# Yelp/nrtsearch

Hardware: AMD Instinct MI355X
Metric: queries/sec, 10M-doc 5-term BM25 top-1000 (higher is better)
Workload: dtype f32

## Files before the change

nrtsearch_amd/csrc/kernels.hip:

```cpp
#include <hip/hip_runtime.h>
#include <stdint.h>

#include "bm25_common.hiph"

namespace nrtgpu {

struct ScanSmem {
  uint64_t acc[kScanWaves][kTileDocs];
  uint64_t cand[kCandCap];
  uint32_t tab[kTabTerms][kTabEntries];
  float    cache[kLdsCaches][256];
  alignas(16) uint32_t w_incl[kScanWaves][kMaxTerms];
  alignas(16) uint32_t w_rec[kScanWaves][kMaxTerms][4];
  uint32_t w_before[kScanWaves][kMaxTerms];
  TopkScratch sc;
  uint64_t theta;
  uint64_t thr;
  uint32_t cnt;
  uint32_t tile_cand;
  uint32_t slot_hits[kSliceSlots];
  uint32_t slot_slice[kSliceSlots];
  uint32_t rz_flag;
  uint32_t cnt_valid;
  uint32_t next_tile;
// ... 714 lines not shown
      hits += h;
      if (h != 0u && q.gte_floor != 0xFFFFFFFFu) atomicAdd(&slice_sum[q.slice_base + s.slot_slice[i]], h);
    }
    item_hits[blockIdx.x] = hits;
    if (ABL == 7 && item_prof) {
      s.prof[4] += __builtin_readcyclecounter() - t_epi;
      for (int i = 0; i < 16; ++i) item_prof[(size_t)blockIdx.x * 16 + i] = s.prof[i];
    }
  }
}

struct MergeSmem {
  uint64_t cand[kMergeCap];
  TopkScratch sc;
  uint64_t theta;
  unsigned long long hits;
  uint32_t cnt;
  uint32_t pad;
  uint32_t lrec[kScanThreads];
  uint32_t loff[kScanThreads + 1];
  uint32_t wtot[kScanThreads / 64];
};

__device__ __noinline__ void merge_compact(MergeSmem& s, uint32_t n, uint32_t k) {
  uint64_t thr = 0;
  const uint32_t m = topk_compact<kScanThreads, kMergeCap>(s.cand, n, k, &s.sc, &thr);
  if (n > k && threadIdx.x == 0) {
    s.cnt = m;
    if (thr > s.theta) s.theta = thr;
  }
  __syncthreads();
}

__global__ __launch_bounds__(kScanThreads)
void merge_topk_kernel(const uint64_t* __restrict__ in_keys, const uint32_t* __restrict__ in_counts,
                       const uint64_t* __restrict__ in_hits, const uint32_t* __restrict__ list_idx,
                       const uint32_t* __restrict__ q_base, const uint32_t* __restrict__ q_nlists, uint32_t k_stride_in,
                       const uint32_t* __restrict__ q_k, uint64_t* __restrict__ out_keys,
                       uint32_t* __restrict__ out_counts, uint64_t* __restrict__ out_hits,
                       uint32_t k_stride_out, const uint32_t* __restrict__ help_query, uint32_t n_help,
                       uint32_t help_slot_base, const unsigned long long* __restrict__ spec_g) {
  __shared__ MergeSmem s;
  const uint32_t tid = threadIdx.x;
  const uint32_t q = blockIdx.x;
  const uint32_t k = q_k[q];
  const uint32_t nl = q_nlists[q];
  const uint32_t base = q_base[q];
  if (tid == 0) {
    s.theta = 0;
    s.hits = 0;
    s.cnt = 0;
  }
  __syncthreads();
  const uint32_t n_lists = nl + (help_query ? n_help : 0u);
  for (uint32_t l0 = 0; l0 < n_lists; l0 += kScanThreads) {
    const uint32_t l = l0 + tid;
    uint32_t rec = 0xFFFFFFFFu, c = 0;
    if (l < nl) {
      rec = list_idx[base + l];
    } else if (l < n_lists && help_query[l - nl] == q + 1u) {
      rec = help_slot_base + (l - nl);
    }
    if (rec != 0xFFFFFFFFu) {
      c = min(in_counts[rec], k_stride_in);
      const unsigned long long h = in_hits[rec];
      if (h) atomicAdd(&s.hits, h);
    }
    const uint32_t incl = scan64_dpp(c);
    const uint32_t lane = tid & 63u, wave = tid >> 6;
    if (lane == 63u) s.wtot[wave] = incl;
    __syncthreads();
    uint32_t before = 0, total = 0;
    for (uint32_t w = 0; w < (uint32_t)(kScanThreads / 64); ++w) {
      const uint32_t t = s.wtot[w];
      before += w < wave ? t : 0u;
      total += t;
    }
    s.lrec[tid] = rec;
    s.loff[tid] = before + incl - c;
    if (tid == 0) s.loff[kScanThreads] = total;
    __syncthreads();
    for (uint32_t i0 = 0; i0 < total; i0 += kScanThreads) {
      const uint32_t i = i0 + tid;
      uint64_t key = 0;
      bool want = false;
      if (i < total) {
        uint32_t lo = 0, hi = kScanThreads;
        while (hi - lo > 1u) {
          const uint32_t mid = (lo + hi) >> 1;
          if (s.loff[mid] <= i) lo = mid; else hi = mid;
        }
        key = in_keys[(size_t)s.lrec[lo] * k_stride_in + (i - s.loff[lo])];
        want = key > s.theta;
      }
      topk_append(s.cand, &s.cnt, want, key);
      __syncthreads();
      const uint32_t cn = s.cnt;
      __syncthreads();
      if (cn > (uint32_t)(kMergeCap - kScanThreads)) merge_compact(s, cn, k);
    }
    __syncthreads();
  }
  __syncthreads();
  {
    const uint32_t c = s.cnt;
    __syncthreads();
    if (c > k) merge_compact(s, c, k);
// ... 175 lines not shown
void launch_pack_write(hipStream_t stream, const uint32_t* docids, const uint32_t* fnorm, uint64_t n, uint32_t n_blocks,
                       const uint32_t* dir, uint32_t* exceptions, uint32_t* packed) {
  if (n_blocks == 0) return;
  hipLaunchKernelGGL(pack_write_kernel, dim3(n_blocks), dim3(256), 0, stream, docids, fnorm, n, dir, exceptions, packed);
}
void launch_apply_live(hipStream_t stream, const uint32_t* docids, uint32_t* fnorm, uint64_t n, const uint64_t* live) {
  if (n == 0) return;
  const uint64_t blocks = (n + 1023) / 1024;
  hipLaunchKernelGGL(apply_live_kernel, dim3((uint32_t)(blocks < 8192 ? blocks : 8192)), dim3(256), 0, stream, docids, fnorm, n, live);
}
void launch_bm25_scan(hipStream_t stream, bool fixed_point, bool pipelined, bool packed, int ablation, uint32_t n_items, const DItem* items,
                      const DPart* parts, const DTerm* terms, const DQuery* queries, const float* caches, unsigned long long* theta_g,
                      unsigned long long* quant_g, const DExchange* xch, uint32_t* slice_sum, uint64_t* item_keys, uint32_t* item_counts,
                      uint64_t* item_hits, uint32_t k_stride, uint64_t* item_prof) {
  if (n_items == 0) return;
#define NRT_LAUNCH_K(F, P, A, K)                                                                                  \
  hipLaunchKernelGGL((bm25_scan_kernel<F, P, A, K>), dim3(n_items), dim3(kScanThreads), 0, stream, items, parts, terms, queries, \
                     caches, theta_g, quant_g, xch, slice_sum, item_keys, item_counts, item_hits, k_stride, item_prof)
#define NRT_LAUNCH(F, P, A)                 \
  do {                                      \
    if (packed) NRT_LAUNCH_K(F, P, A, true);  \
    else NRT_LAUNCH_K(F, P, A, false);      \
  } while (0)
#define NRT_LAUNCH_FX(P, A)            \
  do {                                 \
    if (fixed_point) NRT_LAUNCH(true, P, A); \
    else NRT_LAUNCH(false, P, A);      \
  } while (0)
  if (ablation == 8) { NRT_LAUNCH(true, true, 8); return; }
  if (ablation == 9) { NRT_LAUNCH_FX(true, 9); return; }
  if (!pipelined) { NRT_LAUNCH_FX(false, 0); return; }
  switch (ablation) {
#ifdef NRTGPU_DEV
    case 1: NRT_LAUNCH_K(false, true, 1, false); break;
    case 2: NRT_LAUNCH_K(false, true, 2, false); break;
    case 3: NRT_LAUNCH_K(false, true, 3, false); break;
    case 4: NRT_LAUNCH_K(false, true, 4, false); break;
    case 6: NRT_LAUNCH_K(false, true, 6, false); break;
    case 7: NRT_LAUNCH_FX(true, 7); break;
#endif
    default: NRT_LAUNCH_FX(true, 0); break;
  }
#undef NRT_LAUNCH_FX
#undef NRT_LAUNCH
#undef NRT_LAUNCH_K
}

void launch_merge_topk(hipStream_t stream, uint32_t n_queries, const uint64_t* in_keys, const uint32_t* in_counts,
                       const uint64_t* in_hits, const uint32_t* list_idx, const uint32_t* q_base,
                       const uint32_t* q_nlists, uint32_t k_stride_in, const uint32_t* q_k, uint64_t* out_keys,
                       uint32_t* out_counts, uint64_t* out_hits, uint32_t k_stride_out, const uint32_t* help_query,
                       uint32_t n_help, uint32_t help_slot_base, const unsigned long long* spec_g) {
  if (n_queries == 0) return;
  hipLaunchKernelGGL(merge_topk_kernel, dim3(n_queries), dim3(kScanThreads), 0, stream, in_keys, in_counts, in_hits,
                     list_idx, q_base, q_nlists, k_stride_in, q_k, out_keys, out_counts, out_hits, k_stride_out, help_query, n_help,
                     help_slot_base, spec_g);
}

void launch_fold_norms(hipStream_t stream, const uint32_t* docids, const uint32_t* freqs, const uint8_t* norms,
                       uint32_t* fnorm, uint64_t n, uint32_t* overflow) {
  if (n == 0) return;
  const uint64_t blocks = (n + 255) / 256;
  hipLaunchKernelGGL(fold_norms_kernel, dim3((uint32_t)(blocks < 4096 ? blocks : 4096)), dim3(256), 0, stream, docids,
                     freqs, norms, fnorm, n, overflow);
}

}
```

nrtsearch_amd/csrc/maxscore.hip:

```cpp
#include <hip/hip_runtime.h>
#include <stdint.h>

#include "bm25_common.hiph"

namespace nrtgpu {

constexpr int kMsWinWords = kMsWinDocs / 32;
constexpr int kSl = kMsSlots;
typedef uint32_t u32x2 __attribute__((ext_vector_type(2)));
typedef const NRT_GLOBAL u32x2* gvec2_ptr;

struct alignas(16) WClause {
  uint64_t docids, fnorm;
  uint64_t begin;
  uint32_t count, pad0;
  float    weight;
  int32_t  fx_scale;
  uint32_t flags;
  uint32_t pad;
  uint64_t u_after;
  uint64_t look;
  uint64_t cells, start;
};
static_assert(sizeof(WClause) == 80, "WClause layout");

struct MsSmem {
  uint64_t cand[kMsCandCap];
  uint32_t tab[kTabTerms][kTabEntries];
  float    cache[kLdsCaches][256];
  uint32_t seen[kMsWaves][kMsWinWords];
  WClause  wc[kMsWaves][kMsMaxTerms];
  TopkScratch sc;
  uint64_t theta;
  uint64_t thr;
  uint32_t cnt;
  uint32_t cnt_valid;
  uint32_t rz_flag;
  uint32_t wins_started;
  uint32_t spec_at;
  uint32_t q_wins;
  uint32_t spec_z16;
  uint32_t spec_grow16;
  unsigned long long* spec_slot;
  uint64_t pick;
  uint32_t role[4];
  uint32_t prune_on;
  uint32_t slot_hits[kSliceSlots];
  uint32_t slot_slice[kSliceSlots];
  uint64_t prof[16];
};
static_assert(sizeof(MsSmem) <= 160 * 1024, "the MaxScore workgroup owns one CU's 160 KiB LDS");

__device__ __forceinline__ uint64_t uniform_u64(uint64_t v) {
  const uint32_t lo = (uint32_t)__builtin_amdgcn_readfirstlane((int)(uint32_t)v);
  const uint32_t hi = (uint32_t)__builtin_amdgcn_readfirstlane((int)(uint32_t)(v >> 32));
  return ((uint64_t)hi << 32) | (uint64_t)lo;
}
__device__ __forceinline__ uint64_t readlane_u64(uint64_t v, uint32_t l) {
  const uint32_t lo = (uint32_t)__builtin_amdgcn_readlane((int)(uint32_t)v, (int)l);
  const uint32_t hi = (uint32_t)__builtin_amdgcn_readlane((int)(uint32_t)(v >> 32), (int)l);
  return ((uint64_t)hi << 32) | (uint64_t)lo;
}

template <bool PACKED, int NS>
__device__ __forceinline__ void values_of_codes(const MsSmem& s, const uint32_t (&c)[NS], uint32_t need, uint32_t tab_slot,
                                                float w, int fx_scale, uint32_t cache_slot, uint64_t esc_list,
                                                const uint32_t (&pidx)[NS], uint32_t (&val)[NS]) {
  const uint32_t tab = tab_slot < (uint32_t)kTabTerms ? tab_slot : 7u;
  const char* tb = (const char*)&s.tab[tab == 7u ? 0u : tab][0];
  uint32_t cor = 0;
#pragma unroll
  for (int j = 0; j < NS; ++j) {
    val[j] = *(const uint32_t*)(tb + (c[j] & 0x1FFCu));
    const uint32_t cn = ((need >> j) & 1u) ? c[j] : 0u;
    cor = PACKED ? max(cor, cn) : (cor | cn);
  }
  const bool special = need != 0u && ((PACKED ? cor >= (kPackEscBase << 2) : (cor >> 31) != 0u) || tab == 7u);
  if (__any(special)) {
    const float* cache = &s.cache[cache_slot][0];
#pragma unroll
    for (int j = 0; j < NS; ++j) {
      uint32_t cj = c[j];
      if (PACKED && cj >= (kPackEscBase << 2)) cj = ((need >> j) & 1u) ? packed_escape_word((gu32_ptr)esc_list, pidx[j], cj >> 2) : 0x80000100u;
      const bool esc = (cj >> 31) != 0u;
      const uint32_t f = esc ? ((cj >> 8) & 0x3FFFFFu) : ((cj >> 9) & 15u);
      const bool dead = esc ? ((cj >> 30) & 1u) != 0u : (cj >> 20) != 0u;
      const uint32_t nb = esc ? (cj & 255u) : ((cj >> 2) & 127u);
      if (((need >> j) & 1u) && (esc || tab == 7u))
        val[j] = dead ? 0u : score_value<true>(bm25_score(w, (float)(int32_t)f, cache[nb]), fx_scale);
    }
  }
}

#ifdef NRT_MS_PHASE_CLOCKS
#define NRT_PH_MARK(i)                                                          \
  do {                                                                          \
    if (PROF) {                                                                 \
      asm volatile("s_waitcnt vmcnt(0) lgkmcnt(0)" ::: "memory");               \
      const uint64_t t_ph_ = __builtin_readcyclecounter();                      \
      ph[i] += t_ph_ - ph_t;                                                    \
      ph_t = t_ph_;                                                             \
    }                                                                           \
  } while (0)
#else
// ... 356 lines not shown
        if (lane < n_terms) my_ub = (uint64_t)ub_raw << mt.fx_shift;
      }
      uint64_t my_after = 0;
      {
        uint64_t run = 0;
        for (int m = (int)n_terms - 1; m >= 0; --m) {
          const uint64_t ub = readlane_u64(my_ub, (uint32_t)m);
          if (lane == (uint32_t)m) my_after = run;
          run = use_max ? max(run, ub) : run + ub;
          if (lane == (uint32_t)m) my_suf = run;
        }
      }
      const gu32_ptr my_cells = (gu32_ptr)mt.cell_off;
      const uint32_t my_shift = mt.shift;
      if (lane < n_terms) {
        WClause w;
        w.docids = (uint64_t)mt.docids;
        w.fnorm = (uint64_t)mt.fnorm;
        w.begin = 0;
        w.count = w.pad0 = 0;
        w.weight = mt.weight;
        w.fx_scale = mt.fx_scale;
        const DTermAux* const ax = mt.aux;
        const uint32_t look_kind = ax->look_kind;
        w.flags = ((mt.tab_slot & 0xFFFFu) < (uint32_t)kTabTerms ? (mt.tab_slot & 0xFFFFu) : 7u) | (TWO && (mt.tab_slot & kTabSlotRequired) ? 8u : 0u) |
                  (mt.fx_shift << 4) | (mt.cache_slot << 8) | ((mt.shift & 31u) << 16) | ((look_kind & 7u) << 24) | (((uint32_t)ax->look_shift & 31u) << 27);
        w.pad = 0;
        w.u_after = my_after;
        w.look = look_kind != kLookNone ? (uint64_t)ax->look : 0ull;
        w.cells = (uint64_t)mt.cell_off;
        w.start = mt.start;
        wcl[lane] = w;
      }
      const uint32_t req_mask = TWO ? (uint32_t)__builtin_amdgcn_ballot_w64(lane < n_terms && (mt.tab_slot & kTabSlotRequired) != 0u) : 0u;
      const uint32_t first_req = req_mask != 0u ? (uint32_t)__builtin_ctz(req_mask) : 0xFFu;
      if (PROF) tc_part += __builtin_readcyclecounter() - t_part0;

      for (;;) {
        const uint64_t t_win0 = PROF ? __builtin_readcyclecounter() : 0ull;
        const uint32_t ta = (part.tile_begin & ~(win_tiles - 1u)) + (g - win_base) * win_tiles;
        const uint32_t t0 = max(ta, part.tile_begin);
        const uint32_t t1 = min(ta + win_tiles, part.tile_end);
        const uint32_t doc_lo = t0 * (uint32_t)kTileDocs;
        const uint32_t doc_span = min(t1 * (uint32_t)kTileDocs, part.max_doc) - doc_lo;
        if (PROF) pc_wins += 1;
        if (lane == 0) {
          const uint32_t ws = atomicAdd(&s.wins_started, 1u) + 1u, at = s.spec_at;
          if (at != 0u && ws >= at) __hip_atomic_store(&s.rz_flag, 1u, __ATOMIC_RELAXED, __HIP_MEMORY_SCOPE_WORKGROUP);
        }
        uint32_t g_new = 0;
        if (lane == 0) g_new = (uint32_t)kMsWaves + __hip_atomic_fetch_add(win_next_g, 1u, __ATOMIC_RELAXED, __HIP_MEMORY_SCOPE_AGENT);
        uint64_t theta_other = 0, thr_other = 0;
        if (multi_item) {
          theta_other = __hip_atomic_load(my_theta_g, __ATOMIC_RELAXED, __HIP_MEMORY_SCOPE_AGENT);
          thr_other = acc_threshold<true>(theta_other, fx_E);
          if (mode == kMsModeCount && lane == 0 && __hip_atomic_load(my_prune_g, __ATOMIC_RELAXED, __HIP_MEMORY_SCOPE_AGENT) != 0u)
            __hip_atomic_store(&s.prune_on, 1u, __ATOMIC_RELAXED, __HIP_MEMORY_SCOPE_WORKGROUP);
        }
        uint32_t my_lo = 0, my_hi = 0;
        if (lane < n_terms) {
          my_lo = my_cells[t0 >> my_shift];
          my_hi = my_cells[((t1 - 1u) >> my_shift) + 1u];
        }
        if (n_terms > 1u) {
  #pragma unroll
          for (int j = 0; j < kMsWinWords / 64 / 4; ++j) *(u32x4*)&seen[(lane + 64u * (uint32_t)j) * 4u] = u32x4{0u, 0u, 0u, 0u};
        }
        uint32_t ng = 0;
        {
          const uint64_t thr_w = __hip_atomic_load(&s.prune_on, __ATOMIC_RELAXED, __HIP_MEMORY_SCOPE_WORKGROUP) ? loosen(max(s.thr, thr_other)) : 0ull;
          const uint64_t pb = mt.start + my_lo, pe = mt.start + my_hi;
          if (lane < n_terms) {
            if (my_suf >= thr_w && pe > pb && (!SHAPES || msm <= 1u || lane + msm <= n_terms) && (!TWO || lane <= first_req)) ng = (uint32_t)((pe - (pb & ~3ull) + (uint64_t)(kSl - 1)) / (uint64_t)kSl);
            *(u32x4*)&wcl[lane].begin = u32x4{(uint32_t)pb, (uint32_t)(pb >> 32), (uint32_t)(pe - pb), 0u};
          }
        }
        const uint32_t incl = scan32_dpp(ng);
        uint32_t pre[kMsMaxTerms];
  #pragma unroll
        for (int i = 0; i < kMsMaxTerms; ++i) pre[i] = (uint32_t)__builtin_amdgcn_readlane((int)incl, i);
        const uint32_t n_groups = pre[kMsMaxTerms - 1];

  #ifdef NRT_MS_PHASE_CLOCKS
        if (PROF) ph_t = t_win0;
  #endif
        NRT_PH_MARK(0);
        for (uint32_t v0 = 0; v0 < n_groups; v0 += 64u) {
          const uint32_t v = v0 + lane;
          const bool act = v < n_groups;
          uint32_t c = 0, before = 0;
  #pragma unroll
          for (int i = 0; i < kMsMaxTerms - 1; ++i) {
            c += (v >= pre[i]) ? 1u : 0u;
            before = (v >= pre[i]) ? pre[i] : before;
          }
          const uint32_t c_first = (uint32_t)__builtin_amdgcn_readfirstlane((int)c);
          const uint64_t theta = max(s.theta, theta_other), thr = loosen(max(s.thr, thr_other));
          const bool pruning = __hip_atomic_load(&s.prune_on, __ATOMIC_RELAXED, __HIP_MEMORY_SCOPE_WORKGROUP) != 0u;
          const uint64_t thr_p = pruning ? thr : 0ull;
          if (readlane_u64(my_suf, c_first) < thr_p) break;
          if (PROF) pc_chunks += 1;
          const uint32_t rec = wcl_addr + c * (uint32_t)sizeof(WClause);
          const u32x4 r0 = *(const u32x4*)lds_ptr(rec), r1 = *(const u32x4*)lds_ptr(rec + 16u), r2 = *(const u32x4*)lds_ptr(rec + 32u);
          const uint64_t u_after = *(const uint64_t*)lds_ptr(rec + 48u);
          const uint64_t col_d = ((uint64_t)r0[1] << 32) | r0[0], col_c = ((uint64_t)r0[3] << 32) | r0[2];
          const uint64_t p_begin = ((uint64_t)r1[1] << 32) | r1[0];
          const uint32_t flags = r2[2];
          const uint32_t q0 = (v - before) * (uint32_t)kSl;
          const uint64_t mine0 = (p_begin & ~3ull) + (uint64_t)q0;
          uint32_t d[kSl], cd[kSl];
  #pragma unroll
          for (int j = 0; j < kSl; ++j) d[j] = cd[j] = 0u;
          if (act) {
            const u32x4 d0 = __builtin_nontemporal_load((gvec_ptr)(col_d + mine0 * 4u));
            const u32x4 d1 = kSl > 4 ? __builtin_nontemporal_load((gvec_ptr)(col_d + mine0 * 4u) + 1) : d0;
            if (PACKED) {
              const uint32_t sw = doc_lo & ~kPackDocMask;
  #pragma unroll
              for (int j = 0; j < 4; ++j) {
                d[j] = (d0[j] >> kPackCodeBits) | sw;
                cd[j] = (d0[j] & kPackCodeMask) << 2;
                if (kSl > 4) {
                  d[(4 + j) % kSl] = (d1[j] >> kPackCodeBits) | sw;
                  cd[(4 + j) % kSl] = (d1[j] & kPackCodeMask) << 2;
                }
              }
            } else {
              const u32x4 c0 = __builtin_nontemporal_load((gvec_ptr)(col_c + mine0 * 4u));
              const u32x4 c1 = kSl > 4 ? __builtin_nontemporal_load((gvec_ptr)(col_c + mine0 * 4u) + 1) : c0;
  #pragma unroll
              for (int j = 0; j < 4; ++j) {
                d[j] = d0[j];
                cd[j] = c0[j];
                if (kSl > 4) {
                  d[(4 + j) % kSl] = d1[j];
                  cd[(4 + j) % kSl] = c1[j];
                }
              }
            }
          }
          NRT_PH_MARK(1);
          uint32_t vmask = 0;
          {
            const uint32_t rel = q0 - ((uint32_t)p_begin & 3u), cnt = act ? r1[2] : 0u;
  #pragma unroll
            for (int j = 0; j < kSl; ++j)
              if (rel + (uint32_t)j < cnt && d[j] - doc_lo < doc_span) vmask |= 1u << j;
          }
          uint32_t val[kSl];
          {
            const uint32_t tab = flags & 7u;
            const char* tb = (const char*)&s.tab[tab == 7u ? 0u : tab][0];
            uint32_t cor = 0;
  #pragma unroll
            for (int j = 0; j < kSl; ++j) {
              val[j] = *(const uint32_t*)(tb + (cd[j] & 0x1FFCu));
              const uint32_t cn = ((vmask >> j) & 1u) ? cd[j] : 0u;
              cor = PACKED ? max(cor, cn) : (cor | cn);
            }
            const bool special = vmask != 0u && ((PACKED ? cor >= (kPackEscBase << 2) : (cor >> 31) != 0u) || tab == 7u);
            if (__any(special)) {
              const float w = __uint_as_float(r2[0]);
              const int fx_scale = (int)r2[1];
              const float* cache = &s.cache[(flags >> 8) & 255u][0];
  #pragma unroll
              for (int j = 0; j < kSl; ++j) {
                uint32_t cj = cd[j];
                if (PACKED && cj >= (kPackEscBase << 2))
                  cj = ((vmask >> j) & 1u) ? packed_escape_word((gu32_ptr)col_c, (uint32_t)mine0 + (uint32_t)j, cj >> 2) : 0x80000100u;
                const bool esc = (cj >> 31) != 0u;
                const uint32_t f = esc ? ((cj >> 8) & 0x3FFFFFu) : ((cj >> 9) & 15u);
                const bool dead = esc ? ((cj >> 30) & 1u) != 0u : (cj >> 20) != 0u;
                const uint32_t nb = esc ? (cj & 255u) : ((cj >> 2) & 127u);
                if (((vmask >> j) & 1u) && (esc || tab == 7u))
                  val[j] = dead ? 0u : score_value<true>(bm25_score(w, (float)(int32_t)f, cache[nb]), fx_scale);
              }
            }
          }
          uint64_t run[kSl];
          uint32_t alive = 0;
          {
            const uint32_t mult = 1u << ((flags >> 4) & 15u);
            uint32_t need_v = 1u;
            if (u_after < thr_p) {
              const uint64_t gap = use_max ? thr_p : thr_p - u_after;
              const uint64_t nv = (gap + (uint64_t)(mult - 1u)) >> ((flags >> 4) & 15u);
              need_v = nv > 0xFFFFFFFFull ? 0xFFFFFFFFu : max((uint32_t)nv, 1u);
            }
            uint32_t pass = 0;
  #pragma unroll
            for (int j = 0; j < kSl; ++j) {
              run[j] = (uint64_t)val[j] * (uint64_t)mult;
              pass |= val[j] >= need_v ? (1u << j) : 0u;
            }
            alive = vmask & pass;
            if (need_v == 0xFFFFFFFFu) {
  #pragma unroll
              for (int j = 0; j < kSl; ++j)
                if ((use_max ? max(run[j], u_after) : run[j] + u_after) < thr_p) alive &= ~(1u << j);
            }
          }
          uint64_t sec[TWO ? kSl : 1];
          if (TWO) {
            if ((req_mask & ((1u << c) - 1u)) != 0u) alive = 0u;
            const bool mine_counts = sec_mode == kMsSecTieBreaker || (sec_mode == kMsSecReqOpt && ((req_mask >> c) & 1u) == 0u);
  #pragma unroll
            for (int j = 0; j < kSl; ++j) sec[j] = mine_counts ? run[j] : 0ull;
          }
          if (PROF) {
            pc_post += (uint64_t)__popc(vmask);
            pc_surv += (uint64_t)__popc(alive);
          }
          NRT_PH_MARK(2);
          const uint32_t c_last = (uint32_t)__builtin_amdgcn_readlane((int)c, (int)(min(n_groups - v0, 64u) - 1u));
          if (n_terms > 1u && __any(alive != 0u)) {
            for (uint32_t cc = c_first; cc <= c_last; ++cc) {
              const uint32_t am = c == cc ? alive : 0u;
              if (!__any(am != 0u)) continue;
  #ifdef NRT_MS_COUNT_ROUNDS
              if (PROF) pc_tas += 1;
  #endif
              uint32_t old[kSl];
  #pragma unroll
              for (int j = 0; j < kSl; ++j) {
                const bool a = (am >> j) & 1u;
                const uint32_t w = a ? ((d[j] - doc_lo) >> 5) : lane;
                old[j] = atomicOr(&seen[w], a ? (1u << (d[j] & 31u)) : 0u);
              }
  #pragma unroll
              for (int j = 0; j < kSl; ++j)
                if (((am >> j) & 1u) && ((old[j] >> (d[j] & 31u)) & 1u)) alive &= ~(1u << j);
            }
          }
          NRT_PH_MARK(3);
          uint32_t ccnt = 0x11111111u;

          for (uint32_t j2 = c_first + 1u; j2 < n_terms; ++j2) {
            if (!__any(alive != 0u)) break;
            const uint64_t S_j = readlane_u64(my_suf, j2);
            uint32_t am = c < j2 ? alive : 0u;
            {
              const uint64_t short_of = S_j < thr_p ? (use_max ? thr_p : thr_p - S_j) : 0ull;
              uint32_t kill = 0;
  #pragma unroll
              for (int j = 0; j < kSl; ++j) kill |= run[j] < short_of ? (1u << j) : 0u;
              if (SHAPES && msm > 1u) {
                const uint32_t left = n_terms - j2;
  #pragma unroll
                for (int j = 0; j < kSl; ++j) kill |= ((ccnt >> (4 * j)) & 15u) + left < msm ? (1u << j) : 0u;
              }
              kill &= am;
              alive &= ~kill;
              am &= ~kill;
            }
            if (!__any(am != 0u)) continue;
            if (PROF) pc_look += (uint64_t)__popc(am);
            const WClause& w2 = wcl[j2];
            const uint64_t look2 = uniform_u64(w2.look);
            const uint32_t flags2 = (uint32_t)__builtin_amdgcn_readfirstlane((int)w2.flags);
            const uint32_t kind2 = (flags2 >> 24) & 7u;
            const uint64_t start2 = uniform_u64(w2.start);
            const gu32_ptr codes2 = (gu32_ptr)(uniform_u64(PACKED ? w2.docids : w2.fnorm) + start2 * 4u);
            uint32_t c2[kSl];
            uint32_t pi2[kSl];
            uint32_t present = 0;
  #ifdef NRT_MS_COUNT_ROUNDS
            if (PROF) { if (kind2 == kLookBits) pc_dense += 1; else pc_sparse += 1; }
  #endif
            if (kind2 == kLookBits) {
              const gvec2_ptr recs = (gvec2_ptr)look2;
              u32x2 r[kSl];
  #pragma unroll
              for (int j = 0; j < kSl; ++j) r[j] = recs[((am >> j) & 1u) ? (d[j] >> 5) : 0u];
              __builtin_amdgcn_sched_barrier(0);
              NRT_PH_MARK(4);
              uint32_t idx[kSl];
  #pragma unroll
              for (int j = 0; j < kSl; ++j) {
                const uint32_t bb = d[j] & 31u;
                const bool there = ((am >> j) & 1u) && ((r[j][0] >> bb) & 1u);
                idx[j] = there ? r[j][1] + (uint32_t)__popc(r[j][0] & ((1u << bb) - 1u)) : 0u;
                present |= (there ? 1u : 0u) << j;
              }
  #pragma unroll
              for (int j = 0; j < kSl; ++j) c2[j] = codes2[idx[j]];
              __builtin_amdgcn_sched_barrier(0);
              NRT_PH_MARK(5);
  #pragma unroll
              for (int j = 0; j < kSl; ++j) pi2[j] = (uint32_t)start2 + idx[j];
            } else {
              const gu32_ptr cells2 = (gu32_ptr)(kind2 == kLookCells ? look2 : uniform_u64(w2.cells));
              const gu32_ptr docs2 = (gu32_ptr)(uniform_u64(w2.docids) + start2 * 4u);
              const uint32_t cshift = kind2 == kLookCells ? (flags2 >> 27) & 31u : 10u + ((flags2 >> 16) & 31u);
              uint32_t a[kSl], b[kSl];
  #pragma unroll
// ... 21 lines not shown
  #pragma unroll
                for (int j = 0; j < kSl; ++j)
                  if ((open >> j) & 1u) {
                    const uint32_t dv = PACKED ? vv[j] >> kPackCodeBits : vv[j], dd = PACKED ? d[j] & kPackDocMask : d[j];
                    if (dv < dd) a[j] = mid[j] + 1u;
                    else b[j] = mid[j];
                    if (dv == dd) {
                      a[j] = b[j] = mid[j];
                      present |= 1u << j;
                    }
                    if (!(a[j] < b[j])) open &= ~(1u << j);
                  }
              }
  #pragma unroll
              for (int j = 0; j < kSl; ++j) {
                c2[j] = codes2[((present >> j) & 1u) ? a[j] : 0u];
                pi2[j] = (uint32_t)start2 + a[j];
              }
              NRT_PH_MARK(7);
            }
            if (__any(present != 0u)) {
              uint32_t v2[kSl];
              if (PACKED) {
  #pragma unroll
                for (int j = 0; j < kSl; ++j) c2[j] = (c2[j] & kPackCodeMask) << 2;
              }
              values_of_codes<PACKED, kSl>(s, c2, present, flags2 & 7u, w2.weight, w2.fx_scale, (flags2 >> 8) & 255u, w2.fnorm, pi2, v2);
              const uint32_t mult2 = 1u << ((flags2 >> 4) & 15u);
              if (use_max) {
  #pragma unroll
                for (int j = 0; j < kSl; ++j) run[j] = max(run[j], (uint64_t)(((present >> j) & 1u) ? v2[j] : 0u) * (uint64_t)mult2);
              } else if (TWO && sec_mode != kMsSecNone) {
                const bool counts = sec_mode == kMsSecReqOpt && (flags2 & 8u) == 0u;
  #pragma unroll
                for (int j = 0; j < kSl; ++j) {
                  const uint64_t add = (uint64_t)(((present >> j) & 1u) ? v2[j] : 0u) * (uint64_t)mult2;
                  run[j] += add;
                  sec[j] = sec_mode == kMsSecTieBreaker ? max(sec[j], add) : sec[j] + (counts ? add : 0ull);
                }
              } else {
  #pragma unroll
                for (int j = 0; j < kSl; ++j) run[j] += (uint64_t)(((present >> j) & 1u) ? v2[j] : 0u) * (uint64_t)mult2;
              }
              if (SHAPES && msm > 1u) {
                uint32_t x = present;
                x = (x | (x << 12)) & 0x000F000Fu;
                x = (x | (x << 6)) & 0x03030303u;
                x = (x | (x << 3)) & 0x11111111u;
                ccnt += x;
              }
            }
            if (TWO && (flags2 & 8u) != 0u) alive &= ~(am & ~present);
            NRT_PH_MARK(6);
          }

          {
          uint32_t maybe = 0;
  #pragma unroll
          for (int j = 0; j < kSl; ++j)
            if (((alive >> j) & 1u) && run[j] >= thr) maybe |= 1u << j;
          {
            uint32_t pool = pruning ? maybe : alive;
            if (SHAPES && msm > 1u) {
  #pragma unroll
              for (int j = 0; j < kSl; ++j)
                if (((ccnt >> (4 * j)) & 15u) < msm) pool &= ~(1u << j);
            }
            if (part.live_bits != nullptr && __any(pool != 0u)) {
              uint32_t lw[kSl];
  #pragma unroll
              for (int j = 0; j < kSl; ++j) lw[j] = ((const NRT_GLOBAL uint32_t*)part.live_bits)[((pool >> j) & 1u) ? (d[j] >> 5) : 0u];
  #pragma unroll
              for (int j = 0; j < kSl; ++j)
                if (!((lw[j] >> (d[j] & 31u)) & 1u)) pool &= ~(1u << j);
            }
            maybe &= pool;
            uint32_t h = (uint32_t)__popc(pool);
            h = (uint32_t)__builtin_amdgcn_readlane((int)scan64_dpp(h), 63);
            if (mode == kMsModeCount && !pruning) {
              if (lane == 0 && h != 0u) {
                const uint32_t tot = atomicAdd(&s.slot_hits[cur_slot], h) + h;
                if (tot > q.gte_floor) {
                  __hip_atomic_store(&s.prune_on, 1u, __ATOMIC_RELAXED, __HIP_MEMORY_SCOPE_WORKGROUP);
                  if (multi_item) __hip_atomic_store(my_prune_g, 1u, __ATOMIC_RELAXED, __HIP_MEMORY_SCOPE_AGENT);
                }
              }
            } else {
              wave_hits += h;
            }
          }
          uint64_t theta_now = theta;
          while (__any(maybe != 0u)) {
  #ifdef NRT_MS_COUNT_ROUNDS
            if (PROF) pc_crounds += 1;
  #endif
            const uint32_t low = maybe & (0u - maybe);
            uint64_t rsel = run[0], ssel = TWO ? sec[0] : 0ull;
            uint32_t dsel = d[0];
  #pragma unroll
            for (int j = 1; j < kSl; ++j)
              if (low == (1u << j)) {
                rsel = run[j];
                dsel = d[j];
                if (TWO) ssel = sec[j];
              }
            float score = acc_score<true>(rsel, fx_E);
            if (TWO && sec_mode == kMsSecTieBreaker)
              score = (float)(ldexp((double)ssel, -fx_E) + ldexp((double)(rsel - ssel), -fx_E) * (double)tie_breaker);
            else if (TWO && sec_mode == kMsSecReqOpt)
              score = acc_score<true>(rsel - ssel, fx_E) + acc_score<true>(ssel, fx_E);
            const uint64_t key = pack_key(score, (uint32_t)(part.doc_base + (int32_t)dsel));
            const bool want = low != 0u && key > theta_now && key < after_key;
            uint32_t pos = 0;
            if (!__any(want)) {
              maybe &= ~low;
              continue;
            }
            if (ms_reserve(s, lane, want ? 1u : 0u, pos)) {
              if (want) s.cand[pos] = key;
              if (PROF) pc_cand += want ? 1u : 0u;
              maybe &= ~low;
              continue;
            }
            const uint64_t t_m0 = PROF ? __builtin_readcyclecounter() : 0ull;
            (void)ms_meet(s, k, fx_E, my_theta_g, xch, item.query);
            if (PROF) tc_meet += __builtin_readcyclecounter() - t_m0;
            theta_now = max(theta_now, s.theta);
          }
          }
          NRT_PH_MARK(8);
          if (__hip_atomic_load(&s.rz_flag, __ATOMIC_RELAXED, __HIP_MEMORY_SCOPE_WORKGROUP)) {
            const uint64_t t_m0 = PROF ? __builtin_readcyclecounter() : 0ull;
            (void)ms_meet(s, k, fx_E, my_theta_g, xch, item.query);
            if (PROF) tc_meet += __builtin_readcyclecounter() - t_m0;
          }
        }

        if (PROF) tc_walk += __builtin_readcyclecounter() - t_win0;
        g = window_of_take((uint32_t)__builtin_amdgcn_readfirstlane((int)g_new));
        if (g < win_base || g >= win_base + part_wins) break;
      }
    }
    const uint64_t t_idle0 = PROF ? __builtin_readcyclecounter() : 0ull;
    while (ms_meet(s, k, fx_E, my_theta_g, xch, item.query)) {
    }
    const uint64_t t_epi0 = PROF ? __builtin_readcyclecounter() : 0ull;
    if (PROF && lane == 0) {
      atomicAdd((unsigned long long*)&s.prof[10], (unsigned long long)tc_meet);
      atomicAdd((unsigned long long*)&s.prof[11], (unsigned long long)(t_epi0 - t_idle0));
      atomicAdd((unsigned long long*)&s.prof[12], (unsigned long long)tc_part);
      atomicAdd((unsigned long long*)&s.prof[13], (unsigned long long)(tc_walk - tc_meet));
      atomicMax((unsigned long long*)&s.prof[14], (unsigned long long)(t_idle0 - t_item0));
  #ifdef NRT_MS_COUNT_ROUNDS
      atomicAdd((unsigned long long*)&s.prof[11], (unsigned long long)pc_tas - (unsigned long long)(t_epi0 - t_idle0));
      atomicAdd((unsigned long long*)&s.prof[12], (unsigned long long)pc_dense - (unsigned long long)tc_part);
      atomicAdd((unsigned long long*)&s.prof[10], (unsigned long long)pc_sparse - (unsigned long long)tc_meet);
      atomicAdd((unsigned long long*)&s.prof[13], (unsigned long long)pc_steps - (unsigned long long)(tc_walk - tc_meet));
      atomicAdd((unsigned long long*)&s.prof[8], (unsigned long long)pc_crounds);
  #endif
    }

    {
      const uint32_t c = s.cnt;
      __syncthreads();
      if (c > k) {
        uint64_t thr = 0;
        const uint32_t m = topk_compact<kMsThreads, kMsCandCap>(s.cand, c, k, &s.sc, &thr);
        if (tid == 0) s.cnt = m;
      }
    }
    if (lane == 0 && wave_hits) atomicAdd(&s.slot_hits[cur_slot], wave_hits);
  #ifdef NRT_MS_PHASE_CLOCKS
    if (PROF && lane == 0) {
  #pragma unroll
      for (int i = 0; i < 9; ++i) atomicAdd((unsigned long long*)&s.prof[i], (unsigned long long)ph[i]);
    }
    if (false) {
  #else
    if (PROF && lane == 0) {
      atomicAdd((unsigned long long*)&s.prof[0], (unsigned long long)pc_wins);
      atomicAdd((unsigned long long*)&s.prof[2], (unsigned long long)pc_chunks);
    }
    if (PROF) {
  #endif
      uint64_t v3 = pc_post, v4 = pc_surv, v6 = pc_look, v7 = pc_cand;
  #pragma unroll
      for (int dlt = 32; dlt > 0; dlt >>= 1) {
// ... 216 lines not shown
```

nrtsearch_amd/csrc/search.cpp:

```cpp
#include "runtime_internal.h"


static uint32_t spec_margin16(const nrtgpu_ctx* ctx) { return (uint32_t)std::max(ctx->spec_z16.load(std::memory_order_relaxed), 0); }
static void spec_sync_epoch(const nrtgpu_ctx* ctx, LeafSetCache* lsc) {
  const uint64_t e = ctx->spec_epoch.load(std::memory_order_relaxed);
  if (lsc->spec_epoch.exchange(e, std::memory_order_relaxed) != e) {
    lsc->spec_queries.store(0, std::memory_order_relaxed);
    lsc->spec_reruns.store(0, std::memory_order_relaxed);
    lsc->spec_calls.store(0, std::memory_order_relaxed);
    lsc->spec_calls_rerun.store(0, std::memory_order_relaxed);
    lsc->spec_scattered.store(0, std::memory_order_relaxed);
    lsc->spec_off.store(0, std::memory_order_relaxed);
  }
}
static bool speculating(nrtgpu_ctx* ctx, const nrtgpu_seg* const* segs, int32_t n_segs) {
  if (!ctx || spec_margin16(ctx) == 0u || !segs || n_segs <= 0) return false;
  for (int32_t i = 0; i < n_segs; ++i)
    if (!segs[i]) return false;
  std::shared_ptr<LeafSetCache> lsc = leaf_set_cache(ctx, segs, n_segs);
  spec_sync_epoch(ctx, lsc.get());
  return lsc->spec_off.load(std::memory_order_relaxed) == 0;
}
static void note_speculation_of(nrtgpu_ctx* ctx, LeafSetCache* lsc, int64_t n_queries, int64_t n_rerun) {
  spec_sync_epoch(ctx, lsc);
// ... 74 lines not shown
  if (int rc = slot->d_plan.reserve(plan_bytes)) return rc;
  char* hb = (char*)slot->h_plan.p;
  memcpy(hb + o_queries, hp.queries.data(), hp.queries.size() * sizeof(DQuery));
  if (n_items) memcpy(hb + o_items, hp.items.data(), n_items * sizeof(DItem));
  if (!hp.parts.empty()) memcpy(hb + o_parts, hp.parts.data(), hp.parts.size() * sizeof(DPart));
  if (!hp.qterms.empty()) memcpy(hb + o_qterms, hp.qterms.data(), hp.qterms.size() * sizeof(DQTerm));
  memcpy(hb + o_qexp, hp.qexpand.data(), hp.qexpand.size() * sizeof(DQExpand));
  if (!hp.qs_begin.empty()) memcpy(hb + o_qsb, hp.qs_begin.data(), hp.qs_begin.size() * 4);
  memcpy(hb + o_caches, hp.caches.data(), hp.caches.size() * sizeof(float));
  if (!hp.list_idx.empty()) memcpy(hb + o_lidx, hp.list_idx.data(), hp.list_idx.size() * 4);
  memcpy(hb + o_qbase, hp.q_base.data(), hp.q_base.size() * 4);
  memcpy(hb + o_qnl, hp.q_nlists.data(), hp.q_nlists.size() * 4);
  memcpy(hb + o_qk, hp.q_k.data(), hp.q_k.size() * 4);
  memcpy(hb + o_theta, hp.theta_init.data(), hp.theta_init.size() * 8);
  if (!hp.q_wins.empty()) memcpy(hb + o_qwins, hp.q_wins.data(), hp.q_wins.size() * 4);
  if (spec_world > 1) {
    uint64_t num = (uint64_t)spec_world, den = 1;
    const int64_t sd = ctx->shard_docs.load(std::memory_order_relaxed), id = ctx->index_docs.load(std::memory_order_relaxed);
    if (sd > 0 && id >= sd) {
      num = (uint64_t)id;
      den = (uint64_t)sd;
    }
    uint32_t* qw = (uint32_t*)(hb + o_qwins);
    for (size_t i = 0; i < hp.q_wins.size(); ++i) qw[i] = (uint32_t)std::min<uint64_t>(((uint64_t)qw[i] * num + den - 1) / den, 0xFFFFFFFFull);
  }
  memset(hb + o_quant, 0, hp.list_idx.size() * 8);
  if (ext_hits) memcpy(hb + o_lower, hp.q_lower.data(), hp.q_lower.size() * 8);
  if (use_xch) {
    DExchange x{};
    const size_t stride = (size_t)ctx->cfg.max_batch;
    x.slot = ctx->xch_dev + (size_t)(epoch % kExchangeSlots) * (size_t)ctx->xch_world * stride;
    x.world = (uint32_t)ctx->xch_world;
    x.rank = (uint32_t)ctx->xch_rank;
    x.stride = (uint32_t)stride;
    x.tag = (uint32_t)(epoch + 1);
    if (x.tag == 0) x.tag = 1;
    memcpy(hb + o_xch, &x, sizeof(x));
  }

  static const int env_helpers = (int)dev_env_int("NRTGPU_MS_HELPERS", -1);
  static const int env_help_min = (int)dev_env_int("NRTGPU_MS_HELP_MIN", 16);
  const size_t n_help = hp.n_ms_items == 0 ? 0 : (size_t)(env_helpers >= 0 ? env_helpers : 4 * std::max(ctx->n_cus, 1));
  const size_t n_slots = n_items + n_help;
  Carver wc;
  const size_t o_ikeys = wc.take(n_slots * (size_t)hp.k_stride * 8);
  const size_t o_icnt = wc.take(n_slots * 4);
  const size_t o_ihits = wc.take(n_slots * 8);
  const size_t o_okeys = wc.take((size_t)n_queries * k_stride_out * 8);
  const size_t o_ocnt = wc.take((size_t)n_queries * 4);
  const size_t o_ohits = wc.take((size_t)n_queries * 8);
  const size_t o_terms = wc.take((size_t)hp.n_dterms * sizeof(DTerm));
  const size_t o_ssum = wc.take((size_t)n_queries * hp.n_slices * 4), o_qprune = wc.take((size_t)n_queries * 4);
  const size_t o_hwin = wc.take(hp.n_ms_items * 4), o_hcnt = wc.take(hp.n_ms_items * 4), o_ht0 = wc.take(hp.n_ms_items * 8);
  const size_t o_hhead = wc.take((size_t)n_queries * 4), o_hnext = wc.take(n_help * 4), o_hoff = wc.take(4);
  const size_t o_hqueue = wc.take(4), o_hused = wc.take(4), o_hstart = wc.take(8);
  const uint32_t spec_z16 = spec_margin16(ctx);
  const bool spec = allow_spec && spec_z16 != 0u && hp.n_ms_items != 0 && !use_xch && hp.lsc && hp.lsc->spec_off.load(std::memory_order_relaxed) == 0;
  const size_t o_spec = wc.take(spec ? (size_t)n_queries * 8 : 0);
  const size_t zero_bytes = wc.off - o_ssum;
  const int flag_variant = (ctx->cfg.flags >> 8) & 15;
  const int ablation = hp.clause_counting ? 8 : ((hp.masked && flag_variant == 0 && !(ctx->cfg.flags & NRTGPU_FLAG_NO_MASK_VARIANT)) ? 9 : flag_variant);
  const bool profile = flag_variant == 7;
  const size_t o_prof = wc.take((ablation == 7 || profile) ? n_slots * 128 : 0);
  const size_t o_walls = wc.take(profile ? n_slots * 64 : 0);
  if (int rc = slot->d_work.reserve(wc.off)) return rc;
  char* db = (char*)slot->d_plan.p;
  char* wb = (char*)slot->d_work.p;
  DHelp help{};
  help.win_next = (uint32_t*)(wb + o_hwin);
  help.help_cnt = (uint32_t*)(wb + o_hcnt);
  help.item_t0 = (unsigned long long*)(wb + o_ht0);
  help.help_head = (uint32_t*)(wb + o_hhead);
  help.help_query = (uint32_t*)(wb + o_hnext);
  help.help_off = (uint32_t*)(wb + o_hoff);
  help.item_next = (uint32_t*)(wb + o_hqueue);
  help.help_used = (uint32_t*)(wb + o_hused);
  help.t_start = (unsigned long long*)(wb + o_hstart);
  {
    static const int env_help_alpha = (int)dev_env_int("NRTGPU_MS_HELP_ALPHA", 24);
    uint64_t wins = 0;
    for (size_t i = 0; i < hp.n_ms_items; ++i) wins += hp.items[i].flags >> 8;
    help.total_wins = (uint32_t)std::min<uint64_t>(wins, 0xFFFFFFFFull);
    help.alpha16 = (uint32_t)std::max(env_help_alpha, 0);
    static const int env_spare = (int)dev_env_int("NRTGPU_MS_SPARE_CUS", 8);
    help.n_cus = (uint32_t)std::max(ctx->n_cus - std::max(env_spare, 0), 1);
    if (small) help.n_cus = (uint32_t)std::max(env_spare, 1);
    help.persistent = ms_persistent() ? 1u : 0u;
  }
  help.n_own = (uint32_t)hp.n_ms_items;
  help.n_help = (uint32_t)n_help;
  help.slot_base = (uint32_t)n_items;
  static const bool env_help_greedy = dev_env_int("NRTGPU_MS_HELP_GREEDY", 0) != 0;
  help.min_rem = (uint32_t)std::min(std::max(env_help_min, 1), 0xFFFF) | (env_help_greedy ? 1u << 16 : 0u);
  help.walls = profile ? (unsigned long long*)(wb + o_walls) : nullptr;
  help.spec_g = spec ? (unsigned long long*)(wb + o_spec) : nullptr;
  help.spec_z16 = spec ? spec_z16 : 0u;
  {
    static const int env_first = (int)dev_env_int("NRTGPU_MS_SPEC_FIRST", 2 * kMsWaves);
    static const int env_grow = (int)dev_env_int("NRTGPU_MS_SPEC_GROW", 32);
    help.spec_sched = (uint32_t)std::min(std::max(env_first, 1), 255) | ((uint32_t)std::min(std::max(env_grow, 17), 255) << 8);
  }
  MsArgs ms_args{};
  ms_args.items = (const DItem*)(db + o_items);
  ms_args.parts = (const DPart*)(db + o_parts);
  ms_args.terms = (const DTerm*)(wb + o_terms);
  ms_args.queries = (const DQuery*)(db + o_queries);
  ms_args.caches = (const float*)(db + o_caches);
  ms_args.theta_g = (unsigned long long*)(db + o_theta);
// ... 982 lines not shown
```

Before: 517,300.

## Restructure MaxScore window loop to drain candidates and meet on demand

The merge kernel now scans only as many helper slots as were actually handed out, reading a used-count stored right after the help_query array, instead of all n_help. The MaxScore kernel reorders its LDS struct so the scalars and scratch sit before the large arrays. It also makes thresholds wave-uniform and builds kill masks in registers before applying them. The term loop is restructured so it can break out early when the rendezvous flag is raised, and candidates are drained into a loop that only meets when the buffer is full or rz_flag is set. The aim is to cut wasted merge iterations and reduce scalar/vector traffic and meet latency, but the reworked control flow is intricate and could alter pruning behaviour.

```diff
diff --git a/nrtsearch_amd/csrc/kernels.hip b/nrtsearch_amd/csrc/kernels.hip
--- a/nrtsearch_amd/csrc/kernels.hip
+++ b/nrtsearch_amd/csrc/kernels.hip
@@ -790,7 +790,8 @@
     s.cnt = 0;
   }
   __syncthreads();
-  const uint32_t n_lists = nl + (help_query ? n_help : 0u);
+  const uint32_t n_handed = help_query ? min(help_query[n_help], n_help) : 0u;
+  const uint32_t n_lists = nl + n_handed;
   for (uint32_t l0 = 0; l0 < n_lists; l0 += kScanThreads) {
     const uint32_t l = l0 + tid;
     uint32_t rec = 0xFFFFFFFFu, c = 0;
@@ -1072,6 +1073,7 @@
                        uint32_t* out_counts, uint64_t* out_hits, uint32_t k_stride_out, const uint32_t* help_query,
                        uint32_t n_help, uint32_t help_slot_base, const unsigned long long* spec_g) {
   if (n_queries == 0) return;
+  if (n_help == 0) help_query = nullptr;
   hipLaunchKernelGGL(merge_topk_kernel, dim3(n_queries), dim3(kScanThreads), 0, stream, in_keys, in_counts, in_hits,
                      list_idx, q_base, q_nlists, k_stride_in, q_k, out_keys, out_counts, out_hits, k_stride_out, help_query, n_help,
                      help_slot_base, spec_g);
diff --git a/nrtsearch_amd/csrc/maxscore.hip b/nrtsearch_amd/csrc/maxscore.hip
--- a/nrtsearch_amd/csrc/maxscore.hip
+++ b/nrtsearch_amd/csrc/maxscore.hip
@@ -25,12 +25,6 @@
 static_assert(sizeof(WClause) == 80, "WClause layout");
 
 struct MsSmem {
-  uint64_t cand[kMsCandCap];
-  uint32_t tab[kTabTerms][kTabEntries];
-  float    cache[kLdsCaches][256];
-  uint32_t seen[kMsWaves][kMsWinWords];
-  WClause  wc[kMsWaves][kMsMaxTerms];
-  TopkScratch sc;
   uint64_t theta;
   uint64_t thr;
   uint32_t cnt;
@@ -48,8 +42,17 @@
   uint32_t slot_hits[kSliceSlots];
   uint32_t slot_slice[kSliceSlots];
   uint64_t prof[16];
+  TopkScratch sc;
+  uint64_t cand[kMsCandCap];
+  uint32_t tab[kTabTerms][kTabEntries];
+  float    cache[kLdsCaches][256];
+  uint32_t seen[kMsWaves][kMsWinWords];
+  WClause  wc[kMsWaves][kMsMaxTerms];
 };
 static_assert(sizeof(MsSmem) <= 160 * 1024, "the MaxScore workgroup owns one CU's 160 KiB LDS");
+static_assert(offsetof(MsSmem, seen) % 16 == 0 && offsetof(MsSmem, tab) % 16 == 0 && offsetof(MsSmem, cand) % 16 == 0,
+              "the window bits are cleared, the tables read with 16-byte LDS instructions");
+static_assert(offsetof(MsSmem, cand) < 65536, "the scalars and the selection's scratch lie in front of the arrays: one zero base register");
 
 __device__ __forceinline__ uint64_t uniform_u64(uint64_t v) {
   const uint32_t lo = (uint32_t)__builtin_amdgcn_readfirstlane((int)(uint32_t)v);
@@ -512,8 +515,8 @@
         if (lane == 0) g_new = (uint32_t)kMsWaves + __hip_atomic_fetch_add(win_next_g, 1u, __ATOMIC_RELAXED, __HIP_MEMORY_SCOPE_AGENT);
         uint64_t theta_other = 0, thr_other = 0;
         if (multi_item) {
-          theta_other = __hip_atomic_load(my_theta_g, __ATOMIC_RELAXED, __HIP_MEMORY_SCOPE_AGENT);
-          thr_other = acc_threshold<true>(theta_other, fx_E);
+          theta_other = uniform_u64(__hip_atomic_load(my_theta_g, __ATOMIC_RELAXED, __HIP_MEMORY_SCOPE_AGENT));
+          thr_other = uniform_u64(acc_threshold<true>(theta_other, fx_E));
           if (mode == kMsModeCount && lane == 0 && __hip_atomic_load(my_prune_g, __ATOMIC_RELAXED, __HIP_MEMORY_SCOPE_AGENT) != 0u)
             __hip_atomic_store(&s.prune_on, 1u, __ATOMIC_RELAXED, __HIP_MEMORY_SCOPE_WORKGROUP);
         }
@@ -555,7 +558,7 @@
             before = (v >= pre[i]) ? pre[i] : before;
           }
           const uint32_t c_first = (uint32_t)__builtin_amdgcn_readfirstlane((int)c);
-          const uint64_t theta = max(s.theta, theta_other), thr = loosen(max(s.thr, thr_other));
+          uint64_t thr = uniform_u64(loosen(max(s.thr, thr_other)));
           const bool pruning = __hip_atomic_load(&s.prune_on, __ATOMIC_RELAXED, __HIP_MEMORY_SCOPE_WORKGROUP) != 0u;
           const uint64_t thr_p = pruning ? thr : 0ull;
           if (readlane_u64(my_suf, c_first) < thr_p) break;
@@ -655,9 +658,11 @@
             }
             alive = vmask & pass;
             if (need_v == 0xFFFFFFFFu) {
+              uint32_t shrt = 0;
   #pragma unroll
               for (int j = 0; j < kSl; ++j)
-                if ((use_max ? max(run[j], u_after) : run[j] + u_after) < thr_p) alive &= ~(1u << j);
+                if ((use_max ? max(run[j], u_after) : run[j] + u_after) < thr_p) shrt |= 1u << j;
+              alive &= ~shrt;
             }
           }
           uint64_t sec[TWO ? kSl : 1];
@@ -687,20 +692,27 @@
                 const uint32_t w = a ? ((d[j] - doc_lo) >> 5) : lane;
                 old[j] = atomicOr(&seen[w], a ? (1u << (d[j] & 31u)) : 0u);
               }
+              uint32_t dup = 0;
   #pragma unroll
               for (int j = 0; j < kSl; ++j)
-                if (((am >> j) & 1u) && ((old[j] >> (d[j] & 31u)) & 1u)) alive &= ~(1u << j);
+                if (((am >> j) & 1u) && ((old[j] >> (d[j] & 31u)) & 1u)) dup |= 1u << j;
+              alive &= ~dup;
             }
           }
           NRT_PH_MARK(3);
           uint32_t ccnt = 0x11111111u;
 
-          for (uint32_t j2 = c_first + 1u; j2 < n_terms; ++j2) {
-            if (!__any(alive != 0u)) break;
+          uint32_t j2 = c_first + 1u;
+          for (;;) {
+          for (; j2 < n_terms; ++j2) {
+            if (!__any(alive != 0u)) {
+              j2 = n_terms;
+              break;
+            }
             const uint64_t S_j = readlane_u64(my_suf, j2);
             uint32_t am = c < j2 ? alive : 0u;
             {
-              const uint64_t short_of = S_j < thr_p ? (use_max ? thr_p : thr_p - S_j) : 0ull;
+              const uint64_t short_of = (pruning && S_j < thr) ? (use_max ? thr : thr - S_j) : 0ull;
               uint32_t kill = 0;
   #pragma unroll
               for (int j = 0; j < kSl; ++j) kill |= run[j] < short_of ? (1u << j) : 0u;
@@ -828,9 +840,13 @@
             }
             if (TWO && (flags2 & 8u) != 0u) alive &= ~(am & ~present);
             NRT_PH_MARK(6);
-          }
-
-          {
+            if (__builtin_amdgcn_readfirstlane((int)__hip_atomic_load(&s.rz_flag, __ATOMIC_RELAXED, __HIP_MEMORY_SCOPE_WORKGROUP)) != 0) {
+              ++j2;
+              break;
+            }
+          }
+
+          if (j2 == n_terms) {
           uint32_t maybe = 0;
   #pragma unroll
           for (int j = 0; j < kSl; ++j)
@@ -838,19 +854,22 @@
           {
             uint32_t pool = pruning ? maybe : alive;
             if (SHAPES && msm > 1u) {
+              uint32_t few = 0;
   #pragma unroll
               for (int j = 0; j < kSl; ++j)
-                if (((ccnt >> (4 * j)) & 15u) < msm) pool &= ~(1u << j);
+                if (((ccnt >> (4 * j)) & 15u) < msm) few |= 1u << j;
+              pool &= ~few;
             }
             if (part.live_bits != nullptr && __any(pool != 0u)) {
               uint32_t lw[kSl];
   #pragma unroll
               for (int j = 0; j < kSl; ++j) lw[j] = ((const NRT_GLOBAL uint32_t*)part.live_bits)[((pool >> j) & 1u) ? (d[j] >> 5) : 0u];
-  #pragma unroll
-              for (int j = 0; j < kSl; ++j)
-                if (!((lw[j] >> (d[j] & 31u)) & 1u)) pool &= ~(1u << j);
-            }
-            maybe &= pool;
+              uint32_t in_set = 0;
+  #pragma unroll
+              for (int j = 0; j < kSl; ++j) in_set |= ((lw[j] >> (d[j] & 31u)) & 1u) << j;
+              pool &= in_set;
+            }
+            alive = maybe & pool;
             uint32_t h = (uint32_t)__popc(pool);
             h = (uint32_t)__builtin_amdgcn_readlane((int)scan64_dpp(h), 63);
             if (mode == kMsModeCount && !pruning) {
@@ -865,12 +884,14 @@
               wave_hits += h;
             }
           }
-          uint64_t theta_now = theta;
-          while (__any(maybe != 0u)) {
+          j2 = n_terms + 1u;
+          }
+          bool full = false;
+          while (j2 > n_terms && __any(alive != 0u)) {
   #ifdef NRT_MS_COUNT_ROUNDS
             if (PROF) pc_crounds += 1;
   #endif
-            const uint32_t low = maybe & (0u - maybe);
+            const uint32_t low = alive & (0u - alive);
             uint64_t rsel = run[0], ssel = TWO ? sec[0] : 0ull;
             uint32_t dsel = d[0];
   #pragma unroll
@@ -886,29 +907,29 @@
             else if (TWO && sec_mode == kMsSecReqOpt)
               score = acc_score<true>(rsel - ssel, fx_E) + acc_score<true>(ssel, fx_E);
             const uint64_t key = pack_key(score, (uint32_t)(part.doc_base + (int32_t)dsel));
-            const bool want = low != 0u && key > theta_now && key < after_key;
+            const bool want = low != 0u && key > max(s.theta, theta_other) && key < after_key;
             uint32_t pos = 0;
             if (!__any(want)) {
-              maybe &= ~low;
+              alive &= ~low;
               continue;
             }
             if (ms_reserve(s, lane, want ? 1u : 0u, pos)) {
               if (want) s.cand[pos] = key;
               if (PROF) pc_cand += want ? 1u : 0u;
-              maybe &= ~low;
+              alive &= ~low;
               continue;
             }
+            full = true;
+            break;
+          }
+          NRT_PH_MARK(8);
+          if (full || __builtin_amdgcn_readfirstlane((int)__hip_atomic_load(&s.rz_flag, __ATOMIC_RELAXED, __HIP_MEMORY_SCOPE_WORKGROUP)) != 0) {
             const uint64_t t_m0 = PROF ? __builtin_readcyclecounter() : 0ull;
             (void)ms_meet(s, k, fx_E, my_theta_g, xch, item.query);
             if (PROF) tc_meet += __builtin_readcyclecounter() - t_m0;
-            theta_now = max(theta_now, s.theta);
-          }
-          }
-          NRT_PH_MARK(8);
-          if (__hip_atomic_load(&s.rz_flag, __ATOMIC_RELAXED, __HIP_MEMORY_SCOPE_WORKGROUP)) {
-            const uint64_t t_m0 = PROF ? __builtin_readcyclecounter() : 0ull;
-            (void)ms_meet(s, k, fx_E, my_theta_g, xch, item.query);
-            if (PROF) tc_meet += __builtin_readcyclecounter() - t_m0;
+            thr = uniform_u64(loosen(max(s.thr, thr_other)));
+          }
+          if (j2 > n_terms && !__any(alive != 0u)) break;
           }
         }
 
diff --git a/nrtsearch_amd/csrc/search.cpp b/nrtsearch_amd/csrc/search.cpp
--- a/nrtsearch_amd/csrc/search.cpp
+++ b/nrtsearch_amd/csrc/search.cpp
@@ -150,8 +150,8 @@
   const size_t o_terms = wc.take((size_t)hp.n_dterms * sizeof(DTerm));
   const size_t o_ssum = wc.take((size_t)n_queries * hp.n_slices * 4), o_qprune = wc.take((size_t)n_queries * 4);
   const size_t o_hwin = wc.take(hp.n_ms_items * 4), o_hcnt = wc.take(hp.n_ms_items * 4), o_ht0 = wc.take(hp.n_ms_items * 8);
-  const size_t o_hhead = wc.take((size_t)n_queries * 4), o_hnext = wc.take(n_help * 4), o_hoff = wc.take(4);
-  const size_t o_hqueue = wc.take(4), o_hused = wc.take(4), o_hstart = wc.take(8);
+  const size_t o_hhead = wc.take((size_t)n_queries * 4), o_hnext = wc.take((n_help + 1) * 4), o_hoff = wc.take(4);
+  const size_t o_hqueue = wc.take(4), o_hused = o_hnext + n_help * 4, o_hstart = wc.take(8);
   const uint32_t spec_z16 = spec_margin16(ctx);
   const bool spec = allow_spec && spec_z16 != 0u && hp.n_ms_items != 0 && !use_xch && hp.lsc && hp.lsc->spec_off.load(std::memory_order_relaxed) == 0;
   const size_t o_spec = wc.take(spec ? (size_t)n_queries * 8 : 0);
```

After: 473,800. 8.4% lower.
